# alimt1992/graph-neural-pde

Measured on AMD Instinct MI355X. Metric: ODE RHS evals/s (and ms/step) at |E|≈1.2M, d=128; achieved HBM GB/s vs roofline, higher is better.
Workload: dtype f32; 1 GPU; G-arxiv laplacian RHS, rk4 (configs[2]); nodes=169343, edges=1200000, dim=128, method=rk4, global_batch=1, parallelism=replicas1, chunk=256, node_order=degree, hub_rows=232

## Files before the change

graph-neural-pde_amd/csrc/aggregate.hpp:

```cpp
#pragma once
#include <algorithm>
#include <type_traits>

#include "common.hpp"
#include "scores.hpp"

namespace gnpde {

struct PlainWeights {
  const float* __restrict__ w;
  struct Raw {
    float w;
  };
  __device__ __forceinline__ Raw load(int , int p, int ) const { return Raw{w[p]}; }
  __device__ __forceinline__ float finish(int , const Raw& r) const { return r.w; }
};

template <int MAXH, bool EXACT = false, bool REC = false>
struct RefDstSoftmaxWeights {
  const double* __restrict__ cs;
  const double* __restrict__ m;
  const float* __restrict__ rl;
  int H;
  const float* __restrict__ rec;
// ... 302 lines not shown
  return kWavesPerBlock * RPW * kFrozenPass;
}

template <int VEC, int GL, int RPW>
__device__ __forceinline__ void frozen_tail(const Epi& ep, int C, const float* __restrict__ home, int r0, int r1,
                                            int steps, int tb, int wave, int rs, int gl) {
  const int cc = gl * VEC;
  const int rb = r0 + tb * frozen_rows_per_block<RPW>() + wave * RPW + rs;
  Packed<VEC, float> v[kFrozenPass];
#pragma unroll
  for (int i = 0; i < kFrozenPass; ++i) {
    const int row = rb + i * kWavesPerBlock * RPW;
    if (row < r1 && rs < RPW && cc < C) {
      load_packed<VEC>(home + (int64_t)row * ep.ldx + cc, v[i]);
    } else {
#pragma unroll
      for (int t = 0; t < VEC; ++t) v[i].d[t] = 0u;
    }
  }
  const float a = (ep.flags & GNPDE_EPI_RHS) ? epi_alpha(ep) : 1.f;
  const float sc = out_scale(ep.st, 0, stage_scale(ep.st));
#pragma unroll 1
  for (int k = 1; k < steps; ++k) {
#pragma unroll
    for (int i = 0; i < kFrozenPass; ++i) {
      const Packed<VEC, float> x = v[i];
      float o[VEC], r[VEC];
#pragma unroll
      for (int t = 0; t < VEC; ++t) o[t] = a * (fmaf(1.0f, unpack(x, t), 0.f) - unpack(x, t));
      auto kval = [&](int , int t) -> float { return unpack(x, t); };
      stage_combine<VEC, kStagePre, float>(ep, ep.st.o[0], 0, o, x, &x, kval, sc, r);
      pack_into<VEC, float>(r, v[i]);
    }
  }
#pragma unroll
  for (int i = 0; i < kFrozenPass; ++i) {
    const int row = rb + i * kWavesPerBlock * RPW;
    if (row < r1 && rs < RPW && cc < C) {
      EpiPre<VEC, float, 1> p;
      p.xr = v[i];
      p.x0r = v[i];
#pragma unroll
      for (int j = 0; j < stage_bpre<1>(); ++j) p.base[j] = v[i];
#pragma unroll
      for (int j = 0; j < stage_kpre<1>(); ++j) p.kv[j] = v[i];
      float ax[VEC];
#pragma unroll
      for (int t = 0; t < VEC; ++t) ax[t] = fmaf(1.0f, unpack(v[i], t), 0.f);
      epi_finish<VEC, 1, float>(ep, row, cc, ax, a, 0.f, p, nullptr);
    }
  }
}

template <int VEC, int GL, int NCH, int U, int RPW, int STG_, class WP, class T = float>
__global__ __launch_bounds__(256) void agg_kernel(const int4* __restrict__ items, int n_items, int4* heavy,
                                                   int n_heavy, const int* __restrict__ col, WP wp, int C, Epi ep,
                                                   float* __restrict__ partials, const float* fz_home = nullptr,
                                                   int fz_r0 = 0, int fz_r1 = 0, int fz_steps = 1) {
  constexpr int STG = STG_ == kStgFrozen ? 1 : STG_;
  constexpr int SL = kWave / RPW;
  constexpr int G = SL / GL;
  static_assert((SL & (SL - 1)) == 0 || G == 1, "non-power-of-two row slots hold one edge group");
  constexpr bool PRE = NCH <= 2;
  const int lane = threadIdx.x & 63;
  const int rs = lane / SL, sl = lane % SL;
  const int g = sl / GL, gl = sl % GL;
  if constexpr (STG_ == kStgFrozen) {
    static_assert(NCH == 1 && G == 1 && sizeof(T) == 4, "the frozen tail is written for the headline geometry");
    const int nb = (n_items + kWavesPerBlock * RPW - 1) / (kWavesPerBlock * RPW);
    if ((int)blockIdx.x >= nb) {
      frozen_tail<VEC, GL, RPW>(ep, C, fz_home, fz_r0, fz_r1, fz_steps, (int)blockIdx.x - nb, threadIdx.x >> 6, rs,
                                gl);
      return;
    }
  }
  const int wid = uniform(xcd_block(ep.xcd_remap) * kWavesPerBlock + (threadIdx.x >> 6));
  const int item = wid * RPW + rs;
  if (wid * RPW >= n_items) return;
  const bool live = item < n_items && rs < RPW;
  const int4 it = live ? items[item] : make_int4(0, 0, 0, -1);
  const int row = it.x, beg = it.y, end = it.z, slot = it.w;
  const bool owner = live && slot < 0 && g == 0;

  EpiPre<VEC, T, STG> pre[PRE ? NCH : 1];
  auto prefetch = [&]() {
    if constexpr (PRE) {
      if (owner) {
#pragma unroll
        for (int ch = 0; ch < NCH; ++ch) {
          const int cc = (ch * GL + gl) * VEC;
          if (cc < C) epi_prefetch<VEC, STG, T>(ep, row, cc, pre[ch]);
        }
      }
    }
  };

  float acc[NCH][VEC];
#pragma unroll
  for (int ch = 0; ch < NCH; ++ch)
#pragma unroll
    for (int t = 0; t < VEC; ++t) acc[ch][t] = 0.f;

  constexpr bool SCHED = std::is_same<WP, PlainWeights>::value && sizeof(T) == 4 && VEC == 4 && GL == 32 &&
                         RPW == 2 && NCH == 1 && U == 4;
  if constexpr (SCHED) {
    const int len = end - beg;
// ... 196 lines not shown
        const int cc = (ch * GL + gl) * VEC;
        if (cc < C) epi_prefetch<VEC, STG, T>(ep, erow, cc, pre[ch]);
      }
    }
  }
  const float a = (ep.flags & GNPDE_EPI_RHS) ? epi_alpha(ep) : 1.f;
  const float b = (ep.flags & GNPDE_ADD_SOURCE) ? *ep.beta : 0.f;
  double dpart[2] = {0.0, 0.0};
#pragma unroll
  for (int ch = 0; ch < NCH; ++ch) {
    const int cc = (ch * GL + gl) * VEC;
    if (cc < C) {
      if constexpr (PRE)
        epi_finish<VEC, STG, T>(ep, erow, cc, acc[ch], a, b, pre[ch], dpart);
      else
        epilogue_store<VEC, STG, T>(ep, erow, cc, acc[ch], a, b, dpart);
    }
  }
  if constexpr (stage_rowsum<STG, T>()) {
    const double* prev = nullptr;
    if constexpr (PRE && stage_dot<STG>()) prev = &pre[0].dprev;
    epi_rowsums<GL, STG, T>(ep, erow, dpart, rs * SL, gl == 0, prev);
  }
}

template <int VEC, int GL, int NCH, int U, int RPW, class WP, class T = float>
static int launch_agg_cfg(const int4* items, int64_t n_items, int4* heavy, int64_t n_heavy, const int* col,
                          const WP& wp, int C, const Epi& ep, float* partials, hipStream_t s) {
  const unsigned grid = (unsigned)ceil_div(n_items, (int64_t)kWavesPerBlock * RPW);
  const int nh = (int)n_heavy;
  int stg = epi_stage_kind(ep);
  if (ep.has_stage && ep.st.dense_tab && !ep.st.dense_out) {
    dense_coef_kernel<<<1, kWave, 0, s>>>(ep.st);
    GNPDE_LAUNCH_CHECK();
  }
  if (n_items > 0) {
    if (stg == 3 && !(std::is_same<WP, PlainWeights>::value && sizeof(T) == 4)) stg = 2;
    if (stg == 4) {
      if constexpr (std::is_same<WP, PlainWeights>::value) {
        if (ep.st.dense_out)
          agg_kernel<VEC, GL, NCH, U, RPW, 5, PlainWeights, T><<<grid, kBlock, 0, s>>>(
              items, (int)n_items, heavy, nh, col, as_plain(wp), C, ep, partials);
        else
          agg_kernel<VEC, GL, NCH, U, RPW, 4, PlainWeights, T><<<grid, kBlock, 0, s>>>(
              items, (int)n_items, heavy, nh, col, as_plain(wp), C, ep, partials);
      } else {
        set_error("rhs: the wide (adaptive-solver) stage epilogue is fused with plain weights only; "
                  "apply it with gnpde_stage_apply_*");
        return GNPDE_EUNSUPPORTED;
      }
    } else if (stg == 3)
      agg_kernel<VEC, GL, NCH, U, RPW, 3, PlainWeights, float><<<grid, kBlock, 0, s>>>(
          items, (int)n_items, heavy, nh, col, as_plain(wp), C, ep, partials);
    else if (stg == 1)
      agg_kernel<VEC, GL, NCH, U, RPW, 1, WP, T><<<grid, kBlock, 0, s>>>(items, (int)n_items, heavy, nh, col, wp, C, ep,
                                                                          partials);
    else if (stg == 2)
      agg_kernel<VEC, GL, NCH, U, RPW, 2, WP, T><<<grid, kBlock, 0, s>>>(items, (int)n_items, heavy, nh, col, wp, C, ep,
                                                                          partials);
    else
      agg_kernel<VEC, GL, NCH, U, RPW, 0, WP, T><<<grid, kBlock, 0, s>>>(items, (int)n_items, heavy, nh, col, wp, C, ep,
                                                                          partials);
    GNPDE_LAUNCH_CHECK();
  }
  return GNPDE_OK;
}

template <int VEC, class WP, class T = float>
static int launch_agg_vec(const int4* items, int64_t n_items, int4* heavy, int64_t n_heavy, const int* col,
                          const WP& wp, int C, const Epi& ep, float* partials, hipStream_t s) {
  const int lanes = (int)ceil_div(C, VEC);
#define GNPDE_AGG(GL, NCH, U, RPW) \
  launch_agg_cfg<VEC, GL, NCH, U, RPW, WP, T>(items, n_items, heavy, n_heavy, col, wp, C, ep, partials, s)
  if constexpr (takes_narrow_rows<WP>::value) {
    if (n_items * (int64_t)C * (int64_t)sizeof(T) > (int64_t)(96 << 20)) {
      if (lanes <= 4) return GNPDE_AGG(4, 1, 4, 16);
      if (lanes <= 8) return GNPDE_AGG(8, 1, 4, 8);
      if (lanes <= 16) return GNPDE_AGG(16, 1, 4, 4);
    }
    if (lanes <= 4) return GNPDE_AGG(4, 1, 4, 4);
    if (lanes <= 8) return GNPDE_AGG(8, 1, 8, 4);
    if (lanes <= 16) return GNPDE_AGG(16, 1, 4, 2);
  }
  if (lanes <= 16) return GNPDE_AGG(16, 1, 4, 1);
  if constexpr (sizeof(T) == 2 && VEC == 8) {
    if (lanes > 16 && lanes <= 21) return GNPDE_AGG(21, 1, 4, 3);
  }
  if (lanes <= 32) return GNPDE_AGG(32, 1, 4, 2);
  if (lanes <= 64) return GNPDE_AGG(64, 1, 4, 1);
  if (lanes <= 128) return GNPDE_AGG(64, 2, 2, 1);
  if (lanes <= 256) return GNPDE_AGG(64, 4, 2, 1);
  if (lanes <= 512) return GNPDE_AGG(64, 8, 1, 1);
#undef GNPDE_AGG
  set_error("aggregate: C=%d too wide (max %d)", C, 512 * VEC);
  return GNPDE_EUNSUPPORTED;
}

template <class T = float>
inline int epi_vec_width(const Epi& ep, int64_t C, const void* partials) {
  const int kMax = sizeof(T) == 2 ? ((C > 128 && C <= 256) ? 8 : 4) : 16 / (int)sizeof(T);
  for (int v = kMax; v > 1; v >>= 1) {
    const size_t bytes = (size_t)v * sizeof(T);
    auto al = [&](const void* p) { return p == nullptr || (reinterpret_cast<uintptr_t>(p) % bytes) == 0; };
    bool ok = C % v == 0 && ep.ldx % v == 0 && ep.ldf % v == 0 && al(ep.x);
    if (ep.flags & GNPDE_ADD_SOURCE) ok = ok && ep.ldx0 % v == 0 && al(ep.x0);
    if (ep.has_stage) {
      ok = ok && al(ep.st.f_out);
      for (int i = 0; i < ep.st.n_out; ++i) {
        ok = ok && al(ep.st.o[i].out) && al(ep.st.o[i].base);
      }
      for (int j = 0; j < ep.st.nk; ++j) ok = ok && al(ep.st.k[j]);
      if (ep.st.err_rows) ok = ok && al(ep.st.err.base) && al(ep.st.err_y0);
    } else {
      ok = ok && al(ep.f);
    }
// ... 47 lines not shown
```

graph-neural-pde_amd/csrc/rhs.hip:

```cpp
#include "aggregate.hpp"
#include "rhs_host.hpp"

using namespace gnpde;

extern "C" {

int gnpde_spmm_rhs_f32(const int32_t* items, int64_t n_items, int32_t* heavy, int64_t n_heavy,
                       const int32_t* col, const float* w, int64_t C, const float* x, int64_t ldx, const float* x0,
                       int64_t ldx0, const float* alpha, const float* beta, int flags, float* f, int64_t ldf,
                       float* partials, int64_t n_slots, const gnpde_stage_epilogue_t* stage, void* stream) {
  const Epi ep = make_epi(x, ldx, x0, ldx0, alpha, beta, flags, f, ldf, stage);
  int rc = check_epi(ep, C, n_heavy, partials, n_slots);
  if (rc) return rc;
  GNPDE_REQUIRE(n_items >= 0 && n_items < INT32_MAX && n_heavy >= 0, GNPDE_EINVAL, "spmm_rhs: bad item counts");
  GNPDE_REQUIRE(n_items == 0 || (items && col && w), GNPDE_EINVAL, "spmm_rhs: NULL plan/col/w");
  PlainWeights wp{w};
  return launch_agg(items, n_items, heavy, n_heavy, col, wp, C, ep, partials, as_stream(stream));
}

int gnpde_spmm_rhs_frozen_f32(const int32_t* items, int64_t n_live_items, int32_t* heavy, int64_t n_heavy,
                              const int32_t* col, const float* w, int64_t C, const float* x, int64_t ldx,
                              const float* alpha, int flags, int64_t ldf, float* partials, int64_t n_slots,
                              const gnpde_stage_epilogue_t* stage, const float* home, int64_t row0, int64_t row1,
                              int64_t steps, void* stream) {
  GNPDE_REQUIRE(stage != nullptr && home != nullptr, GNPDE_EINVAL, "spmm_rhs_frozen: NULL stage or home");
  const Epi ep = make_epi(x, ldx, nullptr, 0, alpha, nullptr, flags, nullptr, ldf, stage);
  int rc = check_epi(ep, C, n_heavy, partials, n_slots);
  if (rc) return rc;
  GNPDE_REQUIRE(n_live_items >= 0 && n_live_items < INT32_MAX && n_heavy >= 0, GNPDE_EINVAL,
                "spmm_rhs_frozen: bad item counts");
  GNPDE_REQUIRE(n_live_items == 0 || (items && col && w), GNPDE_EINVAL, "spmm_rhs_frozen: NULL plan/col/w");
  GNPDE_REQUIRE(row0 >= 0 && row0 <= row1 && row1 < INT32_MAX && ldx == ldf, GNPDE_EINVAL,
                "spmm_rhs_frozen: frozen rows [%lld, %lld) / leading dimensions", (long long)row0, (long long)row1);
  GNPDE_REQUIRE(steps >= 1 && steps < INT32_MAX, GNPDE_EINVAL, "spmm_rhs_frozen: steps=%lld", (long long)steps);
  for (int i = 0; i < stage->n_out; ++i)
    GNPDE_REQUIRE(stage->out_rows == nullptr || stage->o[i].out != home, GNPDE_EINVAL,
                  "spmm_rhs_frozen: output %d aliases the frozen rows' home under out_rows", i);
  PlainWeights wp{w};
  return launch_agg_frozen(items, n_live_items, heavy, n_heavy, col, wp, C, ep, partials, home, row0, row1, steps,
                           as_stream(stream));
}

int gnpde_spmm_rhs_bf16(const int32_t* items, int64_t n_items, int32_t* heavy, int64_t n_heavy,
                        const int32_t* col, const float* w, int64_t C, const uint16_t* x, int64_t ldx,
                        const uint16_t* x0, int64_t ldx0, const float* alpha, const float* beta, int flags, uint16_t* f,
                        int64_t ldf, float* partials, int64_t n_slots, const gnpde_stage_epilogue_t* stage,
                        void* stream) {
  GNPDE_REQUIRE(!stage || !stage->dot_rows, GNPDE_EUNSUPPORTED, "spmm_rhs_bf16: stage dot terms are fp32 only");
  const Epi ep = make_epi(reinterpret_cast<const float*>(x), ldx, reinterpret_cast<const float*>(x0), ldx0, alpha,
                          beta, flags, reinterpret_cast<float*>(f), ldf, stage);
  int rc = check_epi(ep, C, n_heavy, partials, n_slots);
  if (rc) return rc;
  GNPDE_REQUIRE(n_items >= 0 && n_items < INT32_MAX && n_heavy >= 0, GNPDE_EINVAL, "spmm_rhs_bf16: bad item counts");
  GNPDE_REQUIRE(n_items == 0 || (items && col && w), GNPDE_EINVAL, "spmm_rhs_bf16: NULL plan/col/w");
  PlainWeights wp{w};
  return launch_agg<PlainWeights, bf16>(items, n_items, heavy, n_heavy, col, wp, C, ep, partials, as_stream(stream));
}

// ... 30 lines not shown
```

graph-neural-pde_amd/gnpde/_lib.py:

```python
import ctypes
import os
import threading

_HERE = os.path.dirname(os.path.abspath(__file__))
LIB_PATH = os.environ.get("GNPDE_LIB", os.path.join(_HERE, "libgnpde.so"))

STAGE_MAX_OUT = 2
STAGE_MAX_K = 6
STAGE_PRE_K = 2
DENSE_BASIS = 5
DENSE_SLOTS = STAGE_MAX_K + 2
ADAMS_MAX_HISTORY = 11


class StageOut(ctypes.Structure):
    _fields_ = [("out", ctypes.c_void_p), ("base", ctypes.c_void_p), ("cb", ctypes.c_float), ("cf", ctypes.c_float),
                ("c", ctypes.c_float * STAGE_MAX_K)]


class StageEpilogue(ctypes.Structure):
    _fields_ = [("f_out", ctypes.c_void_p), ("n_out", ctypes.c_int), ("o", StageOut * STAGE_MAX_OUT),
                ("nk", ctypes.c_int), ("k", ctypes.c_void_p * STAGE_MAX_K),
                ("out_rows", ctypes.c_void_p), ("dot_with", ctypes.c_void_p), ("dot_rows", ctypes.c_void_p),
                ("dot_coef", ctypes.c_double), ("dot_accumulate", ctypes.c_int),
                ("err_rows", ctypes.c_void_p), ("err", StageOut), ("err_y0", ctypes.c_void_p), ("err_y1", ctypes.c_int),
                ("atol", ctypes.c_double), ("rtol", ctypes.c_double), ("coef_scale", ctypes.c_void_p),
                ("f_lin", ctypes.c_float), ("unscaled_outs", ctypes.c_int),
                ("dense_out", ctypes.c_void_p), ("dense_rows", ctypes.c_void_p), ("dense_t", ctypes.c_void_p),
                ("dense_dt", ctypes.c_void_p), ("dense_tab", ctypes.c_void_p),
                ("dense_m", (ctypes.c_float * DENSE_SLOTS) * DENSE_BASIS), ("scale_rows", ctypes.c_void_p)]


c_i32p = ctypes.POINTER(ctypes.c_int32)
c_i64p = ctypes.POINTER(ctypes.c_int64)
_vp = ctypes.c_void_p
_i64 = ctypes.c_int64
_int = ctypes.c_int
_f32 = ctypes.c_float
_f64 = ctypes.c_double
_size = ctypes.c_size_t

SIGNATURES = {
    "gnpde_abi_version": (_int, []),
    "gnpde_last_error": (ctypes.c_char_p, []),
    "gnpde_build_id": (ctypes.c_char_p, []),
    "gnpde_csr_workspace_bytes": (_size, [_i64, _i64, _i64]),
    "gnpde_csr_build": (_int, [_vp, _i64, _i64, _i64, _int, _vp, _vp, _vp, _vp, _size, _vp]),
    "gnpde_gather_weights_f32": (_int, [_vp, _i64, _int, _vp, _vp, _vp]),
    "gnpde_indegree_i32": (_int, [_vp, _i64, _i64, _vp, _vp]),
    "gnpde_mix_weights_f32": (_int, [_vp, _int, _vp, _vp, _i64, _vp, _vp]),
    "gnpde_group_normalize_workspace_bytes": (_size, [_i64]),
    "gnpde_group_normalize_f32": (_int, [_vp, _vp, _i64, _i64, _vp, _vp, _vp, _size, _vp]),
    "gnpde_quantile_workspace_bytes": (_size, [_i64]),
    "gnpde_quantile_f32": (_int, [_vp, _i64, _f64, _vp, _vp, _size, _vp]),
    "gnpde_plan_workspace_bytes": (_size, [_i64]),
    "gnpde_plan_build": (_int, [_vp, _i64, ctypes.c_int32, _vp, _i64, _vp, _i64, c_i64p, c_i64p, c_i64p, _vp,
                                _size, _vp]),
    "gnpde_spmm_rhs_f32": (_int, [_vp, _i64, _vp, _i64, _vp, _vp, _i64, _vp, _i64, _vp, _i64, _vp, _vp, _int, _vp,
                                  _i64, _vp, _i64, ctypes.POINTER(StageEpilogue), _vp]),
    "gnpde_spmm_rhs_frozen_f32": (_int, [_vp, _i64, _vp, _i64, _vp, _vp, _i64, _vp, _i64, _vp, _int, _i64, _vp, _i64,
                                         ctypes.POINTER(StageEpilogue), _vp, _i64, _i64, _i64, _vp]),
    "gnpde_spmm_rhs_bf16": (_int, [_vp, _i64, _vp, _i64, _vp, _vp, _i64, _vp, _i64, _vp, _i64, _vp, _vp, _int, _vp,
                                   _i64, _vp, _i64, ctypes.POINTER(StageEpilogue), _vp]),
    "gnpde_attn_ref_rhs_f32": (_int, [_vp, _i64, _vp, _i64, _vp, _vp, _vp, _vp, _vp, _i64, _i64, _vp, _i64, _vp, _i64,
                                      _vp, _vp, _int, _vp, _i64, _vp, _i64, ctypes.POINTER(StageEpilogue), _vp]),
    "gnpde_attn_dot_supported": (_int, [_i64, _i64, _i64]),
    "gnpde_attn_dot_workspace_floats": (_i64, [_i64, _i64, _i64]),
    "gnpde_attn_dot_rhs_f32": (_int, [_vp, _i64, _vp, _i64, _vp, _vp, _vp, _i64, _i64, _i64, _vp, _i64, _vp, _i64, _vp,
                                      _i64, _vp, _vp, _int, _vp, _i64, _vp, _i64, ctypes.POINTER(StageEpilogue), _vp]),
    "gnpde_attn_dot_rhs_bf16": (_int, [_vp, _i64, _vp, _i64, _vp, _vp, _vp, _i64, _i64, _i64, _vp, _i64, _vp, _i64, _vp,
                                      _i64, _vp, _vp, _int, _vp, _i64, _vp, _i64, ctypes.POINTER(StageEpilogue), _vp]),
    "gnpde_rows_copy": (_int, [_vp, _i64, _i64, _vp, _vp, _vp, _vp]),
    "gnpde_decode_score_f32": (_int, [_vp, _i64, _i64, _i64, _vp, _vp, _i64, _vp, _vp, _vp, _vp, _vp, _vp]),
    "gnpde_threshold_mask_f32": (_int, [_vp, _i64, _vp, _vp, _vp, _vp]),
    "gnpde_initial_step_workspace_bytes": (_size, []),
    "gnpde_adaptive_control": (_int, [_i64, _vp, _f64, _f64, _f64, _f64, _f64, _vp, _vp, _vp, _vp, _vp, _size, _vp]),
    "gnpde_initial_step_f32": (_int, [_i64, _vp, _vp, _vp, _f64, _f64, _f64, _vp, _vp, _vp, _size, _vp]),
    "gnpde_initial_step_rows": (_int, [_i64, _vp, _vp, _f64, _f64, _vp, _vp, _vp, _size, _vp]),
    "gnpde_initial_step_lin_f32": (_int, [_i64, _vp, _vp, _f64, _f64, _f64, _vp, _vp, _vp, _size, _vp]),
    "gnpde_initial_step_lin_bf16": (_int, [_i64, _vp, _vp, _f64, _f64, _f64, _vp, _vp, _vp, _size, _vp]),
    "gnpde_scaled_sq_sums_f32": (_int, [_i64, _vp, _vp, _vp, _f64, _f64, _vp, _vp, _size, _vp]),
    "gnpde_segment_sums_workspace_bytes": (_size, [_i64]),
    "gnpde_segment_sums_f64": (_int, [_i64, _i64, _vp, _vp, _vp, _size, _vp]),
    "gnpde_compact_items_f32": (_int, [_vp, _i64, _vp, _vp, _vp, _vp, _vp, _vp]),
    "gnpde_initial_step_bf16": (_int, [_i64, _vp, _vp, _vp, _f64, _f64, _f64, _vp, _vp, _vp, _size, _vp]),
    "gnpde_stage_apply_f32": (_int, [_i64, _i64, _i64, _vp, _vp, ctypes.POINTER(StageEpilogue), _vp]),
    "gnpde_stage_apply_bf16": (_int, [_i64, _i64, _i64, _vp, _vp, ctypes.POINTER(StageEpilogue), _vp]),
    "gnpde_seg_long_edges": (_int, []),
    "gnpde_seg_long_pass_edges": (_int, [_i64]),
    "gnpde_linear_f32": (_int, [_vp, _i64, _i64, _i64, _vp, _vp, _i64, _i64, _vp, _i64, _vp, _i64, _vp]),
    "gnpde_linear_bf16": (_int, [_vp, _i64, _i64, _i64, _vp, _vp, _i64, _i64, _vp, _i64, _vp, _i64, _vp]),
    "gnpde_linear_rhs_f32": (_int, [_vp, _i64, _i64, _i64, _vp, _i64, _vp, _i64, _vp, _i64, _vp, _vp, _int, _vp, _i64,
                                    ctypes.POINTER(StageEpilogue), _vp]),
    "gnpde_linear_rhs_bias_f32": (_int, [_vp, _i64, _i64, _i64, _vp, _i64, _vp, _vp, _i64, _vp, _i64, _vp, _vp, _int,
                                         _vp, _i64, ctypes.POINTER(StageEpilogue), _vp]),
    "gnpde_head_aggregate_fast": (_int, [_i64, _i64]),
    "gnpde_head_aggregate_workspace_floats": (_i64, [_i64, _i64]),
    "gnpde_head_aggregate_f32": (_int, [_vp, _i64, _vp, _i64, _vp, _vp, _vp, _i64, _vp, _i64, _i64, _vp, _i64, _vp,
                                        _i64, _vp, _i64, _vp]),
    "gnpde_linear_wgrad_workspace_bytes": (_size, [_i64, _i64, _i64]),
    "gnpde_linear_wgrad_f32": (_int, [_vp, _i64, _i64, _i64, _vp, _i64, _i64, _vp, _i64, _vp, _size, _vp]),
    "gnpde_keysum_workspace_bytes": (_size, [_i64, _i64, _i64, _i64]),
    "gnpde_ref_scores_f32": (_int, [_vp, _i64, _i64, _i64, _i64, _vp, _vp, _vp, _vp, _vp, _i64, _i64, _vp, _vp,
                                    _size, _vp]),
    "gnpde_ref_keysum_f32": (_int, [_vp, _i64, _i64, _i64, _i64, _vp, _vp, _vp, _i64, _vp, _vp, _size, _vp]),
    "gnpde_ref_scores_from_keysum_f32": (_int, [_vp, _i64, _i64, _i64, _i64, _vp, _vp, _vp, _i64, _i64, _vp, _vp,
                                                _size, _vp]),
    "gnpde_softmax_stats_f32": (_int, [_vp, _i64, _vp, _i64, _vp, _int, _int, _i64, _i64, _vp, _vp, _vp, _i64, _f32,
                                       _f32, _vp, _vp, _vp, _vp, _vp]),
    "gnpde_attn_weights_f32": (_int, [_vp, _vp, _i64, _int, _int, _i64, _i64, _vp, _vp, _vp, _i64, _f32, _f32, _vp,
                                      _vp, _vp, _vp]),
    "gnpde_edge_attention_f32": (_int, [_vp, _vp, _vp, _i64, _int, _int, _i64, _i64, _vp, _vp, _vp, _i64, _f32, _f32,
                                        _vp, _vp, _vp, _vp]),
    "gnpde_edge_attention_csr_f32": (_int, [_vp, _vp, _i64, _int, _int, _i64, _i64, _vp, _vp, _vp, _i64, _f32, _f32,
# ... 19 lines not shown
    "gnpde_self_loops_workspace_bytes": (_size, [_i64, _i64, _i64]),
    "gnpde_self_loops_count": (_int, [_vp, _i64, _i64, c_i64p, _vp, _size, _vp]),
    "gnpde_add_self_loops": (_int, [_vp, _vp, _i64, _i64, _i64, _f32, _i64, _vp, _vp, _vp, _size, _vp]),
    "gnpde_norm_weights_f32": (_int, [_vp, _vp, _i64, _i64, _i64, _vp, _vp, _int, _vp, _vp, _vp]),
    "gnpde_score_grad_f32": (_int, [_vp, _vp, _vp, _i64, _i64, _int, _int, _i64, _i64, _vp, _vp, _i64, _f32, _f32, _vp,
                                    _vp, _i64, _vp, _vp]),
    "gnpde_score_grad_split_f32": (_int, [_vp, _vp, _vp, _i64, _i64, _int, _i64, _i64, _i64, _vp, _vp, _i64, _f32, _f32,
                                          _vp, _vp, _i64, _vp, _vp]),
    "gnpde_gat_scores_workspace_bytes": (_size, [_i64, _i64]),
    "gnpde_gat_scores_f32": (_int, [_vp, _i64, _i64, _i64, _i64, _vp, _vp, _i64, _i64, _vp, _vp, _size, _vp]),
    "gnpde_attn_gat_rhs_f32": (_int, [_vp, _i64, _vp, _i64, _vp, _vp, _vp, _vp, _int, _i64, _f32, _i64, _vp, _i64, _vp,
                                      _i64, _vp, _vp, _int, _vp, _i64, _vp, _i64, ctypes.POINTER(StageEpilogue), _vp]),
    "gnpde_gat_score_backward_f32": (_int, [_vp, _vp, _vp, _i64, _i64, _vp, _f32, _vp, _vp, _vp]),
    "gnpde_score_max_workspace_bytes": (_size, [_i64]),
    "gnpde_score_max_f32": (_int, [_vp, _vp, _vp, _vp, _i64, _i64, _i64, _int, _i64, _i64, _vp, _vp, _vp, _i64, _f32,
                                   _f32, _vp, _vp, _vp, _vp, _size, _vp]),
    "gnpde_squareplus_stats_f32": (_int, [_vp, _i64, _vp, _i64, _vp, _vp, _int, _i64, _i64, _int, _i64, _vp, _vp, _vp,
                                          _vp, _vp, _vp, _vp]),
    "gnpde_squareplus_weights_f32": (_int, [_vp, _vp, _vp, _i64, _i64, _int, _int, _i64, _vp, _vp, _vp, _vp, _vp,
                                            _vp]),
    "gnpde_squareplus_attention_f32": (_int, [_vp, _vp, _vp, _i64, _i64, _int, _int, _i64, _vp, _vp, _vp, _vp, _vp,
                                              _vp]),
    "gnpde_squareplus_attention_csr_f32": (_int, [_vp, _vp, _vp, _i64, _i64, _int, _int, _i64, _vp, _vp, _vp, _vp,
                                                  _vp, _vp]),
    "gnpde_attn_sp_rhs_f32": (_int, [_vp, _i64, _vp, _i64, _vp, _vp, _vp, _i64, _i64, _vp, _i64, _vp, _i64, _vp, _vp,
                                     _int, _vp, _i64, _vp, _i64, ctypes.POINTER(StageEpilogue), _vp]),
    "gnpde_squareplus_backward_workspace_bytes": (_size, [_i64]),
    "gnpde_squareplus_backward_f32": (_int, [_vp, _vp, _i64, _i64, _i64, _int, _vp, _vp, _vp, _vp, _vp, _vp, _size,
                                             _vp]),
    "gnpde_knn_workspace_bytes": (_size, [_i64, _i64]),
    "gnpde_knn_f32": (_int, [_vp, _i64, _i64, _i64, _i64, _i64, _vp, _vp, _vp, _vp, _vp]),
    "gnpde_cross_attention_f32": (_int, [_vp, _i64, _vp, _vp, _i64, _i64, _i64, _i64, _f32, _vp, _i64, _vp, _vp]),
    "gnpde_adams_predict_f32": (_int, [_i64, _vp, _int, ctypes.POINTER(_vp), ctypes.POINTER(_f64),
                                       ctypes.POINTER(_f64), _vp, _vp, _vp, _vp]),
    "gnpde_adams_workspace_bytes": (_size, []),
    "gnpde_adams_status_reset": (_int, [_vp, _vp]),
    "gnpde_adams_correct_f32": (_int, [_i64, _vp, _vp, _vp, _f64, _f64, _f64, _vp, _vp, _vp, _size, _vp]),
    "gnpde_two_hop_lds_max": (_int, []),
    "gnpde_coalesce_sum_f32": (_int, [_vp, _vp, _vp, _i64, _vp, _vp]),
    "gnpde_two_hop_bound_i32": (_int, [_vp, _vp, _i64, _vp, _vp]),
    "gnpde_two_hop_count_i32": (_int, [_vp, _vp, _i64, _vp, _i64, _i64, _vp, _vp, _vp, _vp]),
    "gnpde_two_hop_fill_f32": (_int, [_vp, _vp, _vp, _i64, _vp, _i64, _i64, _vp, _vp, _vp, _i64, _vp, _vp, _vp, _vp]),
}

ABI_VERSION = 8
OK = 0
EINVAL = -1
EHIP = -2
EUNSUPPORTED = -3
EPI_PLAIN = 0
EPI_RHS = 1
ALPHA_SIGMOID = 2
ADD_SOURCE = 4
SCORE_REFERENCE = 0
SCORE_DOT = 1
SCORE_EXP_KERNEL = 2
SCORE_COSINE = 3
SCORE_PEARSON = 4
SCORE_UNIFORM = 5
SCORE_GAT = 6
NORM_RW_ROW = 0
NORM_RW_COL = 1
NORM_GCN = 2

_lock = threading.Lock()
_lib = None


class GnpdeError(RuntimeError):
    pass


def build_id():
    return load().gnpde_build_id().decode()


def source_hash():
    import importlib.util
    spec = importlib.util.spec_from_file_location("gnpde_srchash", os.path.join(os.path.dirname(_HERE), "srchash.py"))
    mod = importlib.util.module_from_spec(spec)
    spec.loader.exec_module(mod)
    return mod.source_hash()


def load():
    global _lib
    if _lib is not None:
        return _lib
    with _lock:
        if _lib is not None:
            return _lib
        if not os.path.exists(LIB_PATH):
            raise GnpdeError(
                "libgnpde.so not found at %s: build it with `make -C graph-neural-pde_amd` or "
                "`python -c 'import __graft_entry__ as g; g.build()'`" % LIB_PATH)
        lib = ctypes.CDLL(LIB_PATH)
        for name, (res, args) in SIGNATURES.items():
            fn = getattr(lib, name)
            fn.restype = res
            fn.argtypes = args
        ver = lib.gnpde_abi_version()
        if ver != ABI_VERSION:
            raise GnpdeError("libgnpde ABI version %d != expected %d" % (ver, ABI_VERSION))
        _check_fresh(lib)
        _lib = lib
        return lib
# ... 38 lines not shown
```

graph-neural-pde_amd/gnpde/ops.py:

```python
import ctypes
import os

import numpy as np
import torch

from . import _lib
from ._cache import _tensor_key

DEFAULT_CHUNK = int(os.environ.get("GNPDE_CHUNK", 256))
SMALL_GRAPH_ROWS = 50000
SMALL_CHUNK = int(os.environ.get("GNPDE_SMALL_CHUNK", 16))


SEG_LONG_SPLIT = os.environ.get("GNPDE_SEG_LONG_SPLIT", "1") != "0"


def auto_chunk(R, chunk=None):
    if chunk is not None:
        return int(chunk)
    if "GNPDE_CHUNK" in os.environ:
        return DEFAULT_CHUNK
    return SMALL_CHUNK if R < SMALL_GRAPH_ROWS else DEFAULT_CHUNK
STATS_CHUNK = 64
PLAN_ORDER = os.environ.get("GNPDE_PLAN_ORDER", "classes")
# ... 641 lines not shown
    lr = _rows(like, "stage rows", dt)
    R, C = lr.shape
    for t in stage.tensors() + [v for v in (f, x) if v is not None]:
        _require_gpu(t, "stage tensor", dt)
        if not t.is_contiguous() or t.numel() != lr.numel():
            raise ValueError("stage tensors must be contiguous and shaped alike")
    st = stage.struct(x, like=lr)
    name = "gnpde_stage_apply_bf16" if dt == torch.bfloat16 else "gnpde_stage_apply_f32"
    _lib.call(name, R, C, C, _ptr(f), _ptr(x), ctypes.byref(st), _stream(lr.device))


def spmm_rhs(g, w_csr, x, x0=None, alpha=None, beta=None, rhs=True, alpha_sigmoid=True, add_source=False,
             out=None, transpose=False, stage=None, frozen=None):
    on_the_fly = (RefDstWeights, GatWeights, RefDstSquareplusWeights)
    if stage is not None and stage.wide and isinstance(w_csr, on_the_fly):
        f = spmm_rhs(g, w_csr, x, x0=x0, alpha=alpha, beta=beta, rhs=rhs, alpha_sigmoid=alpha_sigmoid,
                     add_source=add_source, transpose=transpose)
        stage_apply(stage, f, x, x)
        return None
    shape = x.shape
    dt = x.dtype if isinstance(x, torch.Tensor) and x.dtype in STATE_DTYPES else torch.float32
    xr = _rows(x, "x", dt)
    C = xr.shape[1]
    if xr.shape[0] != g.R:
        raise ValueError("x has %d rows, graph has %d" % (xr.shape[0], g.R))
    dev = xr.device
    a = _scalar(alpha, "alpha", dev) if rhs else None
    if rhs and a is None:
        raise ValueError("spmm_rhs: alpha required")
    b = _scalar(beta, "beta", dev) if add_source else None
    x0r = _rows(x0, "x0", dt) if add_source else None
    st = None
    if stage is not None:
        for t in stage.tensors():
            _require_gpu(t, "stage tensor", dt)
            if not t.is_contiguous() or t.numel() != xr.numel():
                raise ValueError("stage tensors must be contiguous and shaped like x")
        st = ctypes.byref(stage.struct(xr))
    elif out is None:
        out = torch.empty_like(xr)
    grouped = g.csc if transpose else g.csr
    plan = grouped.plan
    partials = _partials(plan, C, dev)
    plan.order_launch(dev)
    epi = (C, _ptr(xr), C, _ptr(x0r), C, _ptr(a), _ptr(b), _flags(rhs, alpha_sigmoid, add_source), _ptr(out), C,
           _ptr(partials), plan.n_slots, st, _stream(dev))
    items, col = plan.items, grouped.col
    if frozen is not None:
        fr, home, steps = frozen
        if (fr.plan is not plan or stage is None or dt != torch.float32 or not isinstance(w_csr, torch.Tensor)
                or add_source or not rhs):
            raise ValueError("spmm_rhs: frozen rows take the plain-weight fp32 stage launches of their own graph")
        if home is None:
            _lib.call("gnpde_spmm_rhs_f32", _ptr(items), fr.n_live_items, _ptr(plan.heavy), plan.n_heavy,
                      _ptr(col), _ptr(w_csr), *epi)
        else:
            hr = _rows(home, "frozen home", dt)
            if hr.shape != xr.shape:
                raise ValueError("spmm_rhs: the frozen rows' home must be shaped like x")
            _lib.call("gnpde_spmm_rhs_frozen_f32", _ptr(items), fr.n_live_items, _ptr(plan.heavy), plan.n_heavy,
                      _ptr(col), _ptr(w_csr), C, _ptr(xr), C, _ptr(a), _flags(rhs, alpha_sigmoid, add_source), C,
                      _ptr(partials), plan.n_slots, st, _ptr(hr), fr.n_live, fr.n_rows, int(steps), _stream(dev))
        return None
    if isinstance(w_csr, CompactWeights):
        if w_csr.grouped is not grouped or w_csr.transpose != bool(transpose):
            raise ValueError("spmm_rhs: compacted weights of another grouped CSR")
        items, col, w_csr = w_csr.items, w_csr.col, w_csr.w
    if dt == torch.bfloat16:
        if isinstance(w_csr, on_the_fly):
            raise ValueError("bf16 storage takes precomputed weights (attn_rhs(..., fuse=False))")
        _lib.call("gnpde_spmm_rhs_bf16", _ptr(items), plan.n_items, _ptr(plan.heavy), plan.n_heavy,
                  _ptr(col), _ptr(w_csr), *epi)
    elif isinstance(w_csr, RefDstWeights):
        if transpose:
            raise ValueError("on-the-fly attention weights aggregate over the CSR only")
        _lib.call("gnpde_attn_ref_rhs_f32", _ptr(plan.items), plan.n_items, _ptr(plan.heavy), plan.n_heavy,
                  _ptr(grouped.col), _ptr(w_csr.cs), _ptr(w_csr.m), _ptr(w_csr.rl), _ptr(w_csr.mr), w_csr.heads,
                  *epi)
    elif isinstance(w_csr, GatWeights):
        if transpose:
            raise ValueError("on-the-fly attention weights aggregate over the CSR only")
        _lib.call("gnpde_attn_gat_rhs_f32", _ptr(plan.items), plan.n_items, _ptr(plan.heavy), plan.n_heavy,
                  _ptr(grouped.col), _ptr(w_csr.sp), _ptr(w_csr.m), _ptr(w_csr.rl), w_csr.norm_idx, w_csr.heads,
                  w_csr.slope, *epi)
    elif isinstance(w_csr, RefDstSquareplusWeights):
        if transpose:
            raise ValueError("on-the-fly attention weights aggregate over the CSR only")
        _lib.call("gnpde_attn_sp_rhs_f32", _ptr(plan.items), plan.n_items, _ptr(plan.heavy), plan.n_heavy,
                  _ptr(grouped.col), _ptr(w_csr.pn), _ptr(w_csr.rl), w_csr.heads, *epi)
    else:
        _lib.call("gnpde_spmm_rhs_f32", _ptr(items), plan.n_items, _ptr(plan.heavy), plan.n_heavy,
                  _ptr(col), _ptr(w_csr), *epi)
    return None if stage is not None else out.view(shape)


class CompactWeights(object):

    def __init__(self, grouped, transpose, full, col, w, items):
        self.grouped, self.transpose = grouped, transpose
        self.full, self.col, self.w, self.items = full, col, w, items


def compact_weights(grouped, w_full, transpose, out=None):
    plan = grouped.plan
    dev = w_full.device
    _require_gpu(w_full, "w_full", torch.float32)
    if out is None:
        out = CompactWeights(grouped, transpose, w_full, torch.empty_like(grouped.col),
# ... 1427 lines not shown
```

include/gnpde.h:

```cpp
#ifndef GNPDE_H_
#define GNPDE_H_

#include <stddef.h>
#include <stdint.h>

#ifdef __cplusplus
extern "C" {
#endif

#define GNPDE_ABI_VERSION 8

#define GNPDE_OK 0
#define GNPDE_EINVAL (-1)
#define GNPDE_EHIP (-2)
#define GNPDE_EUNSUPPORTED (-3)

#define GNPDE_EPI_PLAIN 0
#define GNPDE_EPI_RHS 1
#define GNPDE_ALPHA_SIGMOID 2
#define GNPDE_ADD_SOURCE 4

#define GNPDE_SCORE_REFERENCE 0
#define GNPDE_SCORE_DOT 1
#define GNPDE_SCORE_EXP_KERNEL 2
#define GNPDE_SCORE_COSINE 3
#define GNPDE_SCORE_PEARSON 4
#define GNPDE_SCORE_UNIFORM 5
#define GNPDE_SCORE_GAT 6

int gnpde_abi_version(void);
const char* gnpde_last_error(void);
const char* gnpde_build_id(void);

size_t gnpde_csr_workspace_bytes(int64_t B, int64_t E, int64_t N);
int gnpde_csr_build(const int64_t* edge_index, int64_t B, int64_t E, int64_t N, int key_row,
                    int32_t* rowptr, int32_t* col, int32_t* perm,
                    void* workspace, size_t workspace_bytes, void* stream);

int gnpde_csr_rowidx(const int32_t* rowptr, int64_t R, int64_t nnz, int32_t* rowidx, void* stream);

int gnpde_gather_weights_f32(const float* w_in, int64_t nnz, int H, const int32_t* perm, float* w_out,
                             void* stream);

int gnpde_mix_weights_f32(const float* att, int H, const float* ew, const float* gamma, int64_t n, float* out,
                          void* stream);

size_t gnpde_group_normalize_workspace_bytes(int64_t nnz);
int gnpde_group_normalize_f32(const int32_t* rowptr, const int32_t* perm, int64_t R, int64_t nnz, const float* w_in,
                              float* w_out, void* workspace, size_t workspace_bytes, void* stream);

size_t gnpde_quantile_workspace_bytes(int64_t n);
int gnpde_quantile_f32(const float* v, int64_t n, double q, float* out, void* workspace, size_t workspace_bytes,
                       void* stream);

int gnpde_threshold_mask_f32(const float* v, int64_t n, const float* thr, float* out, int64_t* count, void* stream);
int gnpde_compact_items_f32(const int32_t* items, int64_t n_items, const int32_t* col, const float* w,
                            int32_t* col_out, float* w_out, int32_t* items_out, void* stream);

int gnpde_indegree_i32(const int32_t* idx, int64_t nnz, int64_t R, int32_t* deg, void* stream);

#define GNPDE_NORM_RW_ROW 0
#define GNPDE_NORM_RW_COL 1
#define GNPDE_NORM_GCN 2
size_t gnpde_self_loops_workspace_bytes(int64_t B, int64_t E, int64_t N);
int gnpde_self_loops_count(const int64_t* edge_index, int64_t B, int64_t E, int64_t* nonloop, void* workspace,
                           size_t workspace_bytes, void* stream);
int gnpde_add_self_loops(const int64_t* edge_index, const float* w, int64_t B, int64_t E, int64_t N, float fill,
                         int64_t K, int64_t* ei_out, float* w_out, void* workspace, size_t workspace_bytes,
                         void* stream);
int gnpde_norm_weights_f32(const int64_t* edge_index, const float* w, int64_t B, int64_t E, int64_t N,
                           const int32_t* rowptr, const int32_t* perm, int mode, float* fac, float* w_out,
                           void* stream);

// ... 11 lines not shown
  const float* base;
  float cb;
  float cf;
  float c[GNPDE_STAGE_MAX_K];
} gnpde_stage_out_t;

typedef struct {
  float* f_out;
  int n_out;
  gnpde_stage_out_t o[GNPDE_STAGE_MAX_OUT];
  int nk;
  const float* k[GNPDE_STAGE_MAX_K];
  const int32_t* out_rows;
  const float* dot_with;
  double* dot_rows;
  double dot_coef;
  int dot_accumulate;
  double* err_rows;
  gnpde_stage_out_t err;
  const float* err_y0;
  int err_y1;
  double atol;
  double rtol;
  const float* coef_scale;
  float f_lin;
  int unscaled_outs;
  float* const* dense_out;
  const int32_t* dense_rows;
  const double* dense_t;
  const double* dense_dt;
  float* dense_tab;
  float dense_m[GNPDE_DENSE_BASIS][GNPDE_STAGE_MAX_K + 2];
  double* scale_rows;
} gnpde_stage_epilogue_t;

int gnpde_stage_apply_f32(int64_t R, int64_t C, int64_t ld, const float* f, const float* x,
                          const gnpde_stage_epilogue_t* stage, void* stream);
int gnpde_stage_apply_bf16(int64_t R, int64_t C, int64_t ld, const uint16_t* f, const uint16_t* x,
                           const gnpde_stage_epilogue_t* stage, void* stream);

int gnpde_spmm_rhs_f32(const int32_t* items, int64_t n_items, int32_t* heavy, int64_t n_heavy,
                       const int32_t* col, const float* w, int64_t C,
                       const float* x, int64_t ldx, const float* x0, int64_t ldx0,
                       const float* alpha, const float* beta, int flags,
                       float* f, int64_t ldf, float* partials, int64_t n_slots,
                       const gnpde_stage_epilogue_t* stage, void* stream);

int gnpde_spmm_rhs_frozen_f32(const int32_t* items, int64_t n_live_items, int32_t* heavy, int64_t n_heavy,
                              const int32_t* col, const float* w, int64_t C, const float* x, int64_t ldx,
                              const float* alpha, int flags, int64_t ldf, float* partials, int64_t n_slots,
                              const gnpde_stage_epilogue_t* stage, const float* home, int64_t row0, int64_t row1,
                              int64_t steps, void* stream);

int gnpde_spmm_rhs_bf16(const int32_t* items, int64_t n_items, int32_t* heavy, int64_t n_heavy,
                        const int32_t* col, const float* w, int64_t C, const uint16_t* x, int64_t ldx,
                        const uint16_t* x0, int64_t ldx0, const float* alpha, const float* beta, int flags, uint16_t* f,
                        int64_t ldf, float* partials, int64_t n_slots, const gnpde_stage_epilogue_t* stage,
                        void* stream);

#define GNPDE_STATS_RECORD_FLOATS(h) ((2 * (h) + 3) & ~3)
int gnpde_attn_ref_rhs_f32(const int32_t* items, int64_t n_items, int32_t* heavy, int64_t n_heavy,
                           const int32_t* col, const double* cs, const double* m, const float* rl, const float* mr,
                           int64_t heads,
                           int64_t C, const float* x, int64_t ldx, const float* x0, int64_t ldx0, const float* alpha,
                           const float* beta, int flags, float* f, int64_t ldf, float* partials, int64_t n_slots,
                           const gnpde_stage_epilogue_t* stage, void* stream);

int gnpde_attn_dot_supported(int64_t heads, int64_t dk, int64_t C);
int64_t gnpde_attn_dot_workspace_floats(int64_t heads, int64_t C, int64_t n_slots);
int gnpde_attn_dot_rhs_f32(const int32_t* items, int64_t n_items, int32_t* heavy, int64_t n_heavy,
                           const int32_t* col, const float* q, const float* k, int64_t ldqk, int64_t heads, int64_t dk,
                           const float* dst_stats, int64_t C, const float* x, int64_t ldx, const float* x0, int64_t ldx0,
                           const float* alpha, const float* beta, int flags, float* f, int64_t ldf, float* workspace,
                           int64_t n_slots, const gnpde_stage_epilogue_t* stage, void* stream);
int gnpde_attn_dot_rhs_bf16(const int32_t* items, int64_t n_items, int32_t* heavy, int64_t n_heavy,
                            const int32_t* col, const float* q, const float* k, int64_t ldqk, int64_t heads,
                            int64_t dk, const float* dst_stats, int64_t C, const void* x, int64_t ldx, const void* x0,
                            int64_t ldx0, const float* alpha, const float* beta, int flags, void* f, int64_t ldf,
                            float* workspace, int64_t n_slots, const gnpde_stage_epilogue_t* stage, void* stream);

int gnpde_linear_f32(const float* x, int64_t R, int64_t K, int64_t ldx, const float* W, const float* bias,
                     int64_t Nout, int64_t split, float* out_a, int64_t lda, float* out_b, int64_t ldb,
                     void* stream);
int gnpde_linear_bf16(const void* x, int64_t R, int64_t K, int64_t ldx, const float* W, const float* bias,
                      int64_t Nout, int64_t split, float* out_a, int64_t lda, float* out_b, int64_t ldb,
                      void* stream);

int gnpde_linear_rhs_f32(const float* z, int64_t R, int64_t K, int64_t ldz,
                         const float* Wt , int64_t C,
                         const float* x, int64_t ldx, const float* x0, int64_t ldx0,
                         const float* alpha, const float* beta, int flags,
                         float* f, int64_t ldf,
                         const gnpde_stage_epilogue_t* stage, void* stream);

int gnpde_linear_rhs_bias_f32(const float* z, int64_t R, int64_t K, int64_t ldz,
                              const float* Wt , int64_t C, const float* bias,
                              const float* x, int64_t ldx, const float* x0, int64_t ldx0,
                              const float* alpha, const float* beta, int flags,
                              float* f, int64_t ldf,
                              const gnpde_stage_epilogue_t* stage, void* stream);

int gnpde_head_aggregate_fast(int64_t heads, int64_t dk);
int64_t gnpde_head_aggregate_workspace_floats(int64_t dk, int64_t n_slots);
int gnpde_head_aggregate_f32(const int32_t* items, int64_t n_items, int32_t* heavy, int64_t n_heavy,
                             const int32_t* rowptr, const int32_t* col, const int32_t* perm, int64_t R,
                             const float* w, int64_t heads, int64_t dk, const float* v, int64_t ldv,
// ... 212 lines not shown
```

Measured before the change: 13520 RHS evals/s.

## Add column-striped SpMM kernel mapping feature stripes to XCD groups

Adds a striped aggregation kernel that splits the feature dimension into 2 or 4 column stripes and assigns each stripe to a subset of XCDs. Each XCD's L2 then holds only its slice of the gathered x table, which should improve cache hit rates for random neighbor gathers. Hub rows get a cross-stripe ticket completion. The striped path is enabled by default only for stage kind 1 with the new LIVE_ITEMS flag (set on the frozen-rows path) and a large enough table. The price is redundant col/w index loads per stripe and some extra complexity in the hub completion.

```diff
diff --git a/graph-neural-pde_amd/csrc/aggregate.hpp b/graph-neural-pde_amd/csrc/aggregate.hpp
--- a/graph-neural-pde_amd/csrc/aggregate.hpp
+++ b/graph-neural-pde_amd/csrc/aggregate.hpp
@@ -378,6 +378,151 @@
   }
 }
 
+int k1_stripes_for(int64_t n_items, int64_t C, int stage_kind, int flags);
+void k1_striped_launched();
+
+template <int VEC, int GL, int NCH, int U, int RPW, int STG, class WP, class T>
+constexpr bool striped_geometry() {
+  return std::is_same<WP, PlainWeights>::value && sizeof(T) == 4 && VEC == 4 && GL == 32 && RPW == 2 && NCH == 1 &&
+         U == 4 && (STG == 0 || STG == 1);
+}
+
+template <int S>
+constexpr int stripe_rpw() {
+  return 2 * S;
+}
+template <int S>
+inline unsigned stripe_grid(int64_t n_items) {
+  const int64_t nib = ceil_div(n_items, (int64_t)kWavesPerBlock * stripe_rpw<S>());
+  return (unsigned)(ceil_div(nib, (int64_t)(kNumXcd / S)) * kNumXcd);
+}
+
+template <int S, int STG>
+__global__ __launch_bounds__(256) void agg_stripe_kernel(const int4* __restrict__ items, int n_items, int4* heavy,
+                                                          int n_heavy, const int* __restrict__ col, PlainWeights wp,
+                                                          int C, Epi ep, float* __restrict__ partials) {
+  static_assert((S == 2 || S == 4) && (STG == 0 || STG == 1), "stripes of the forward epilogues");
+  static_assert(!stage_rowsum<STG, float>(), "no per-row term to reduce across stripes");
+  constexpr int VEC = 4, U = 8;
+  constexpr int SL = 32 / S;
+  constexpr int KR = 1;
+  constexpr int RPW = stripe_rpw<S>();
+  constexpr int XS = kNumXcd / S;
+  const int b = blockIdx.x;
+  const int stripe = (b % kNumXcd) / XS;
+  const int ib = (b / kNumXcd) * XS + b % XS;
+  const int c0 = stripe * SL * VEC;
+  if (c0 >= C) return;
+  const int lane = threadIdx.x & 63;
+  const int rs = lane / SL, gl = lane % SL;
+  const int wid = uniform(ib * kWavesPerBlock + (threadIdx.x >> 6));
+  if (wid * RPW >= n_items) return;
+  const int item = wid * RPW + rs;
+  const bool live = item < n_items;
+  const int4 it = live ? items[item] : make_int4(0, 0, 0, -1);
+  const int row = it.x, beg = it.y, end = it.z, slot = it.w;
+  const int cc = c0 + gl * VEC;
+  const bool inc = cc < C;
+  const bool owner = live && slot < 0 && inc;
+
+  EpiPre<VEC, float, STG> pre;
+  if (owner) epi_prefetch<VEC, STG, float>(ep, row, cc, pre);
+  float acc[VEC];
+#pragma unroll
+  for (int t = 0; t < VEC; ++t) acc[t] = 0.f;
+  const float* __restrict__ xb = ep.x + cc;
+  constexpr int CH = KR * SL;
+  for (int e0 = beg; e0 < end; e0 += CH) {
+    const int n = min(CH, end - e0);
+    int mc[KR];
+    float mw[KR];
+#pragma unroll
+    for (int k = 0; k < KR; ++k) {
+      const int e = k * SL + gl;
+      mc[k] = 0;
+      mw[k] = 0.f;
+      if (e < n) {
+        mc[k] = col[e0 + e];
+        mw[k] = wp.w[e0 + e];
+      }
+    }
+#pragma unroll
+    for (int k = 0; k < KR; ++k) {
+      const int nk = min(SL, n - k * SL);
+#pragma unroll
+      for (int j = 0; j < SL; j += U) {
+        if (j >= nk) break;
+        Packed<VEC, float> v[U];
+        float ww[U];
+        int srcl[U];
+#pragma unroll
+        for (int u = 0; u < U; ++u) {
+          const int jj = j + u;
+          const int src = rs * SL + (jj < nk ? jj : 0);
+          srcl[u] = src;
+          const int c = __shfl(mc[k], src);
+          if (jj < nk && inc) {
+            load_packed<VEC>(xb + (int64_t)c * ep.ldx, v[u]);
+          } else {
+#pragma unroll
+            for (int t = 0; t < VEC; ++t) v[u].d[t] = 0u;
+          }
+        }
+#pragma unroll
+        for (int u = 0; u < U; ++u) {
+          const float wsl = __shfl(mw[k], srcl[u]);
+          ww[u] = j + u < nk ? wsl : 0.f;
+        }
+#pragma unroll
+        for (int u = 0; u < U; ++u)
+#pragma unroll
+          for (int t = 0; t < VEC; ++t) acc[t] = fmaf(ww[u], unpack(v[u], t), acc[t]);
+      }
+    }
+  }
+
+  const bool chunk = live && slot >= 0;
+  const bool anyc = n_heavy > 0 && __ballot(chunk) != 0;
+  if (anyc && chunk) {
+    const __amdgpu_buffer_rsrc_t rp = buf_rsrc(partials);
+    buf_store_wt<VEC>(rp, inc ? (uint32_t)(((int64_t)slot * C + cc) * 4) : kBufNone, acc);
+  }
+  const float a = (ep.flags & GNPDE_EPI_RHS) ? epi_alpha(ep) : 1.f;
+  const float bt = (ep.flags & GNPDE_ADD_SOURCE) ? *ep.beta : 0.f;
+  if (owner) epi_finish<VEC, STG, float>(ep, row, cc, acc, a, bt, pre, nullptr);
+  if (!anyc) return;
+
+  asm volatile("s_waitcnt vmcnt(0)" ::: "memory");
+  const int nstr = (C + SL * VEC - 1) / (SL * VEC);
+  int lo = 0, won = 0;
+  if (chunk) {
+    int hi = n_heavy - 1;
+    while (lo < hi) {
+      const int mid = (lo + hi + 1) >> 1;
+      if (heavy[mid].y <= slot)
+        lo = mid;
+      else
+        hi = mid - 1;
+    }
+    if (gl == 0) {
+      const int t = __hip_atomic_fetch_add(&heavy[lo].w, 1, kHubTicketOrder, __HIP_MEMORY_SCOPE_AGENT);
+      won = t == heavy[lo].z * nstr - 1;
+    }
+  }
+#pragma unroll 1
+  for (int s = 0; s < RPW; ++s) {
+    if (__shfl(won, s * SL)) {
+      const int h = __shfl(lo, s * SL);
+      __builtin_amdgcn_fence(__ATOMIC_ACQUIRE, "agent");
+      const int4 hv = heavy[h];
+      float hs[1][VEC];
+      hub_sum<VEC, 32, 1>(uniform(hv.y), uniform(hv.z), C, partials, hs);
+      if (lane < 32 && lane * VEC < C) epilogue_store<VEC, STG, float>(ep, uniform(hv.x), lane * VEC, hs[0], a, bt);
+      if (lane == 0) __hip_atomic_store(&heavy[h].w, 0, __ATOMIC_RELAXED, __HIP_MEMORY_SCOPE_AGENT);
+    }
+  }
+}
+
 template <int VEC, int GL, int NCH, int U, int RPW, int STG_, class WP, class T = float>
 __global__ __launch_bounds__(256) void agg_kernel(const int4* __restrict__ items, int n_items, int4* heavy,
                                                    int n_heavy, const int* __restrict__ col, WP wp, int C, Epi ep,
@@ -680,15 +825,34 @@
     } else if (stg == 3)
       agg_kernel<VEC, GL, NCH, U, RPW, 3, PlainWeights, float><<<grid, kBlock, 0, s>>>(
           items, (int)n_items, heavy, nh, col, as_plain(wp), C, ep, partials);
-    else if (stg == 1)
-      agg_kernel<VEC, GL, NCH, U, RPW, 1, WP, T><<<grid, kBlock, 0, s>>>(items, (int)n_items, heavy, nh, col, wp, C, ep,
-                                                                          partials);
     else if (stg == 2)
       agg_kernel<VEC, GL, NCH, U, RPW, 2, WP, T><<<grid, kBlock, 0, s>>>(items, (int)n_items, heavy, nh, col, wp, C, ep,
                                                                           partials);
-    else
-      agg_kernel<VEC, GL, NCH, U, RPW, 0, WP, T><<<grid, kBlock, 0, s>>>(items, (int)n_items, heavy, nh, col, wp, C, ep,
-                                                                          partials);
+    else {
+      int stripes = 0;
+      if constexpr (striped_geometry<VEC, GL, NCH, U, RPW, 0, WP, T>()) stripes = k1_stripes_for(n_items, C, stg, ep.flags);
+      if (stripes) {
+        if constexpr (striped_geometry<VEC, GL, NCH, U, RPW, 0, WP, T>()) {
+#define GNPDE_STRIPED(S, STG)                                                                                       \
+  agg_stripe_kernel<S, STG><<<stripe_grid<S>(n_items), kBlock, 0, s>>>(items, (int)n_items, heavy, nh, col, wp, C, ep, \
+                                                                        partials)
+          if (stripes == 4) {
+            if (stg == 1) GNPDE_STRIPED(4, 1);
+            else GNPDE_STRIPED(4, 0);
+          } else {
+            if (stg == 1) GNPDE_STRIPED(2, 1);
+            else GNPDE_STRIPED(2, 0);
+          }
+#undef GNPDE_STRIPED
+          k1_striped_launched();
+        }
+      } else if (stg == 1)
+        agg_kernel<VEC, GL, NCH, U, RPW, 1, WP, T><<<grid, kBlock, 0, s>>>(items, (int)n_items, heavy, nh, col, wp, C,
+                                                                            ep, partials);
+      else
+        agg_kernel<VEC, GL, NCH, U, RPW, 0, WP, T><<<grid, kBlock, 0, s>>>(items, (int)n_items, heavy, nh, col, wp, C,
+                                                                            ep, partials);
+    }
     GNPDE_LAUNCH_CHECK();
   }
   return GNPDE_OK;
diff --git a/graph-neural-pde_amd/csrc/rhs.hip b/graph-neural-pde_amd/csrc/rhs.hip
--- a/graph-neural-pde_amd/csrc/rhs.hip
+++ b/graph-neural-pde_amd/csrc/rhs.hip
@@ -1,9 +1,53 @@
 #include "aggregate.hpp"
 #include "rhs_host.hpp"
 
+#include <atomic>
+#include <cstdlib>
+
 using namespace gnpde;
 
+namespace {
+std::atomic<int> g_stripes_set{-1};
+std::atomic<long long> g_striped_launches{0};
+
+int stripes_env() {
+  static const int v = [] {
+    const char* e = std::getenv("GNPDE_K1_STRIPES");
+    if (!e || !*e) return -1;
+    const int s = std::atoi(e);
+    return (s == 0 || s == 2 || s == 4) ? s : -1;
+  }();
+  return v;
+}
+}
+
+namespace gnpde {
+constexpr int kStripesDefault = 2;
+constexpr int64_t kStripeMinTableBytes = (int64_t)65536 * 128 * sizeof(float);
+
+int k1_stripes_for(int64_t n_items, int64_t C, int stage_kind, int flags) {
+  const int set = g_stripes_set.load(std::memory_order_relaxed);
+  const int mode = set >= 0 ? set : stripes_env();
+  if (mode >= 0) return mode;
+  return stage_kind == 1 && (flags & GNPDE_LIVE_ITEMS) && n_items * C * (int64_t)sizeof(float) >= kStripeMinTableBytes ? kStripesDefault : 0;
+}
+void k1_striped_launched() { g_striped_launches.fetch_add(1, std::memory_order_relaxed); }
+}
+
 extern "C" {
+
+int gnpde_k1_stripes_set(int stripes) {
+  GNPDE_REQUIRE(stripes == -1 || stripes == 0 || stripes == 2 || stripes == 4, GNPDE_EINVAL,
+                "k1_stripes_set: stripes=%d not in {-1, 0, 2, 4}", stripes);
+  g_stripes_set.store(stripes, std::memory_order_relaxed);
+  return GNPDE_OK;
+}
+
+int gnpde_k1_stripes_for(int64_t n_items, int64_t C, int stage_kind, int flags) {
+  return k1_stripes_for(n_items, C, stage_kind, flags);
+}
+
+int64_t gnpde_k1_striped_launches(void) { return (int64_t)g_striped_launches.load(std::memory_order_relaxed); }
 
 int gnpde_spmm_rhs_f32(const int32_t* items, int64_t n_items, int32_t* heavy, int64_t n_heavy,
                        const int32_t* col, const float* w, int64_t C, const float* x, int64_t ldx, const float* x0,
diff --git a/graph-neural-pde_amd/gnpde/_lib.py b/graph-neural-pde_amd/gnpde/_lib.py
--- a/graph-neural-pde_amd/gnpde/_lib.py
+++ b/graph-neural-pde_amd/gnpde/_lib.py
@@ -60,6 +60,9 @@
                                   _i64, _vp, _i64, ctypes.POINTER(StageEpilogue), _vp]),
     "gnpde_spmm_rhs_frozen_f32": (_int, [_vp, _i64, _vp, _i64, _vp, _vp, _i64, _vp, _i64, _vp, _int, _i64, _vp, _i64,
                                          ctypes.POINTER(StageEpilogue), _vp, _i64, _i64, _i64, _vp]),
+    "gnpde_k1_stripes_set": (_int, [_int]),
+    "gnpde_k1_stripes_for": (_int, [_i64, _i64, _int, _int]),
+    "gnpde_k1_striped_launches": (_i64, []),
     "gnpde_spmm_rhs_bf16": (_int, [_vp, _i64, _vp, _i64, _vp, _vp, _i64, _vp, _i64, _vp, _i64, _vp, _vp, _int, _vp,
                                    _i64, _vp, _i64, ctypes.POINTER(StageEpilogue), _vp]),
     "gnpde_attn_ref_rhs_f32": (_int, [_vp, _i64, _vp, _i64, _vp, _vp, _vp, _vp, _vp, _i64, _i64, _vp, _i64, _vp, _i64,
@@ -185,6 +188,7 @@
 EPI_RHS = 1
 ALPHA_SIGMOID = 2
 ADD_SOURCE = 4
+LIVE_ITEMS = 8
 SCORE_REFERENCE = 0
 SCORE_DOT = 1
 SCORE_EXP_KERNEL = 2
diff --git a/graph-neural-pde_amd/gnpde/ops.py b/graph-neural-pde_amd/gnpde/ops.py
--- a/graph-neural-pde_amd/gnpde/ops.py
+++ b/graph-neural-pde_amd/gnpde/ops.py
@@ -717,8 +717,9 @@
                 or add_source or not rhs):
             raise ValueError("spmm_rhs: frozen rows take the plain-weight fp32 stage launches of their own graph")
         if home is None:
+            live = epi[:7] + (epi[7] | _lib.LIVE_ITEMS,) + epi[8:]
             _lib.call("gnpde_spmm_rhs_f32", _ptr(items), fr.n_live_items, _ptr(plan.heavy), plan.n_heavy,
-                      _ptr(col), _ptr(w_csr), *epi)
+                      _ptr(col), _ptr(w_csr), *live)
         else:
             hr = _rows(home, "frozen home", dt)
             if hr.shape != xr.shape:
diff --git a/include/gnpde.h b/include/gnpde.h
--- a/include/gnpde.h
+++ b/include/gnpde.h
@@ -19,6 +19,7 @@
 #define GNPDE_EPI_RHS 1
 #define GNPDE_ALPHA_SIGMOID 2
 #define GNPDE_ADD_SOURCE 4
+#define GNPDE_LIVE_ITEMS 8
 
 #define GNPDE_SCORE_REFERENCE 0
 #define GNPDE_SCORE_DOT 1
@@ -136,6 +137,10 @@
                               const gnpde_stage_epilogue_t* stage, const float* home, int64_t row0, int64_t row1,
                               int64_t steps, void* stream);
 
+int gnpde_k1_stripes_set(int stripes);
+int gnpde_k1_stripes_for(int64_t n_items, int64_t C, int stage_kind, int flags);
+int64_t gnpde_k1_striped_launches(void);
+
 int gnpde_spmm_rhs_bf16(const int32_t* items, int64_t n_items, int32_t* heavy, int64_t n_heavy,
                         const int32_t* col, const float* w, int64_t C, const uint16_t* x, int64_t ldx,
                         const uint16_t* x0, int64_t ldx0, const float* alpha, const float* beta, int flags, uint16_t* f,
```

Measured after the change: 15580 RHS evals/s, median of 6. 1.15x the previous value.
